# aantropov/Sailor

Measured on AMD Instinct MI355X. Metric: lit Mpixels/s (K0+K1 tile light cull + K2 PBR shade over per-tile lists), higher is better.
Workload: dtype f32; 1 GPU; C3: 3840x2160, 65536 point+spot lights, 16x16 tiles (240x135), cull + PBR shade; width=3840, height=2160, lights=65536, parallelism=tile-row bands x1, partition=whole frame

## Files before the change

sailor_amd/csrc/light_cull.hip:

```cpp
#include "common.h"
#include "light_record.h"
#include <vector>

#define BANDS_PER_BLOCK 24
#define MAX_BANDS_PER_BLOCK 256
#define QCAP 128
#define GROUP 4
#define CAPG 2048
#define GROUP_OVERFLOW 0xFFFFFFFFu
#define GROUP_OVERFLOW_LISTED 0xFFFFFFFEu
#define GROUP_LISTED 0x40000000u
#define HEAVY_MIN_FRAME 512
#define HEAVY_MIN_BAND 384
#define HEAVY_MAX 96
#define CHUNK 512

#define PACK_TILES 64
#define SEL_LIGHTS 1024
#define CL_STEPS (CAPG / 4 / 64)

#define BAND_FORM_MAX_TILES 12000

struct CullLayout {
    int Tx, Ty, bandRows, bandTiles, numBands, words, groupsX, groupsY, numGroups, packBlocks;
// ... 354 lines not shown
        x = L->worldPosition[0]; y = L->worldPosition[1]; z = L->worldPosition[2]; radius = L->bounds[0];
        type = L->type;
    }
}
__device__ __forceinline__ float4 select_view(const SelectArgs& a, const float x, const float y, const float z, const float radius)
{
    float4 p = glsl_mul(a.view, x, y, z, 1.0f);
    const float w = p.w;
    p.x = p.x / w; p.y = p.y / w; p.z = p.z / w;
    p.z = p.z * -1.0f;
    return make_float4(p.x, p.y, p.z, radius);
}

__global__ __launch_bounds__(256) void k0_band_count(const SelectArgs a)
{
    __shared__ float4 sPl[2];
    __shared__ uint32_t sCnt[4][4];
    const int lane = threadIdx.x & 63, wave = threadIdx.x >> 6;
    const uint32_t b = blockIdx.x;
    if (threadIdx.x == 0) {
        Frustum4 f;
        frustum_from_rect(a.invProj, 0.0f, (float)(a.tileRow0 * TILE), (float)(a.Tx * TILE), (float)((a.tileRow0 + a.bandRows) * TILE), a.vpW, a.vpH, f);
        sPl[0] = make_float4(f.n[2][0], f.n[2][1], f.n[2][2], 0.0f);
        sPl[1] = make_float4(f.n[3][0], f.n[3][1], f.n[3][2], 0.0f);
    }
    float4 lv[4];
    uint32_t type[4];
#pragma unroll
    for (int k = 0; k < 4; k++) {
        const int j = (int)b * SEL_LIGHTS + k * 256 + (int)threadIdx.x;
        lv[k] = make_float4(0.0f, 0.0f, 0.0f, 0.0f);
        type[k] = 1u;
        if (j < a.N) {
            float x, y, z, radius;
            if (a.prepStaged) {
                const float4* L = reinterpret_cast<const float4*>(a.lights + j);
                const float4 q0 = L[0], q1 = L[1], q2 = L[2], q3 = L[3], q4 = L[4], q5 = L[5], q6 = L[6];
                x = q1.x; y = q1.y; z = q1.z; radius = q6.x;
                type[k] = __float_as_uint(q0.x);
                a.prepPosRadius[j] = make_float4(x, y, z, radius);
                a.prepType[j] = type[k];
                if (!a.stageSelectedOnly) {
                    float4 o0, o1, o2, o3, o4;
                    stage_light_record(q0, q1, q2, q3, q4, q5, q6, o0, o1, o2, o3, o4);
                    float4* o = a.prepStaged + (size_t)j * LREC;
                    o[0] = o0; o[1] = o1; o[2] = o2; o[3] = o3; o[4] = o4;
                }
            } else select_load(a, j, x, y, z, radius, type[k]);
            lv[k] = select_view(a, x, y, z, radius);
        }
    }
    __syncthreads();
#pragma unroll
    for (int k = 0; k < 4; k++) {
        const int j = (int)b * SEL_LIGHTS + k * 256 + (int)threadIdx.x;
        const bool valid = j < a.N;
        const float r = lv[k].w;
        const float m = a.planeMargin * ((fabsf(lv[k].x) + fabsf(lv[k].y)) + (fabsf(lv[k].z) + fabsf(r)));
        const bool inFront = (lv[k].z - r) > m;
        const float thr = -(r + m);
        const bool keepAlways = valid && (type[k] == 0u || !inFront);
        const float4 nA = sPl[0], nB = sPl[1];
        const bool out = dot3f(nA.x, nA.y, nA.z, lv[k].x, lv[k].y, lv[k].z) < thr || dot3f(nB.x, nB.y, nB.z, lv[k].x, lv[k].y, lv[k].z) < thr;
        const unsigned long long keep = __ballot(keepAlways || (valid && !out));
        if (lane == 0) { a.keep[(size_t)b * 16u + (uint32_t)(4 * k + wave)] = keep; sCnt[k][wave] = (uint32_t)__popcll(keep); }
    }
    __syncthreads();
    if (threadIdx.x == 0) {
        uint32_t total = 0u;
#pragma unroll
        for (int k = 0; k < 4; k++)
#pragma unroll
            for (int w = 0; w < 4; w++) total += sCnt[k][w];
        a.state[2u + b] = total;
    }
}

__global__ __launch_bounds__(256) void k0_band_scatter(const SelectArgs a)
{
    __shared__ uint32_t sPart[4];
    const int lane = threadIdx.x & 63, wave = __builtin_amdgcn_readfirstlane((int)(threadIdx.x >> 6));
    const uint32_t b = blockIdx.x;
    unsigned long long keep[4];
    uint32_t before[4], total = 0u;
#pragma unroll
    for (int k = 0; k < 4; k++) {
        before[k] = total;
#pragma unroll
        for (int w = 0; w < 4; w++) {
            const unsigned long long m = a.keep[(size_t)b * 16u + (uint32_t)(4 * k + w)];
            const uint32_t c = (uint32_t)__popcll(m);
            if (w == wave) keep[k] = m;
            if (w < wave) before[k] += c;
            total += c;
        }
    }
    uint32_t acc = 0u;
    for (uint32_t i = threadIdx.x; i < b; i += 256u) acc += a.state[2u + i];
#pragma unroll
    for (int d = 32; d > 0; d >>= 1) acc += (uint32_t)__shfl_xor((int)acc, d, 64);
    if (lane == 0) sPart[wave] = acc;
    __syncthreads();
    const uint32_t base = (sPart[0] + sPart[1]) + (sPart[2] + sPart[3]);
    if (b == gridDim.x - 1u && threadIdx.x == 0) a.state[0] = base + total;
#pragma unroll
    for (int k = 0; k < 4; k++) {
        if ((keep[k] >> lane) & 1ull) {
            const uint32_t c = base + before[k] + (uint32_t)__popcll(keep[k] & lanemask_lt());
            const int j = (int)b * SEL_LIGHTS + k * 256 + (int)threadIdx.x;
            float x, y, z, radius;
            uint32_t type;
            if (a.prepStaged) {
                const float4 pr = a.prepPosRadius[j];
                x = pr.x; y = pr.y; z = pr.z; radius = pr.w;
                type = a.prepType[j];
            } else select_load(a, j, x, y, z, radius, type);
            a.lightView[c] = select_view(a, x, y, z, radius);
            a.lightType[c] = type;
            a.lightMap[c] = (uint32_t)j;
            if (a.prepStaged && a.stageSelectedOnly) {
                const float4* L = reinterpret_cast<const float4*>(a.lights + j);
                float4 o0, o1, o2, o3, o4;
                stage_light_record(L[0], L[1], L[2], L[3], L[4], L[5], L[6], o0, o1, o2, o3, o4);
                float4* o = a.prepStaged + (size_t)j * LREC;
                o[0] = o0; o[1] = o1; o[2] = o2; o[3] = o3; o[4] = o4;
            }
        }
    }
}

#define LDS_K01_PREPARE (2 * MAX_BANDS_PER_BLOCK * 16)
#ifndef CULL_SGPR_CAP_PREPARE
#define CULL_SGPR_CAP_PREPARE 96
#endif
__global__ __launch_bounds__(256) __attribute__((amdgpu_num_sgpr(CULL_SGPR_CAP_PREPARE))) void k01_prepare(PrepareArgs a)
{
    __shared__ __attribute__((aligned(16))) unsigned char lds[LDS_K01_PREPARE];
    const int b = (int)blockIdx.x;
    if (b == 0 && threadIdx.x == 0) a.heavy[0] = 0u;
    if (b < a.lightRoleBlocks) k0_lights(b, lds, a);
    else if (b < a.lightRoleBlocks + a.frustumBlocks) k1_tile_frusta(b - a.lightRoleBlocks, a);
    else k1_tile_setup(b - a.lightRoleBlocks - a.frustumBlocks, lds, a);
}

__device__ __forceinline__ uint64_t lanemask_lt()
{
    const uint32_t lane = threadIdx.x & 63;
    return lane == 0 ? 0ull : (~0ull >> (64 - lane));
}

#define WAVE_SYNC() __builtin_amdgcn_fence(__ATOMIC_ACQ_REL, "workgroup")

#define GL_WPT 4
__global__ __launch_bounds__(256) void k1_group_lists(const unsigned long long* __restrict__ masks, const unsigned long long* __restrict__ dirWords,
                                                       int stride, int groupsX, uint32_t* __restrict__ groupCount, uint32_t* __restrict__ groupList,
                                                       uint32_t* __restrict__ heavy, uint32_t heavyMin, const uint32_t* __restrict__ selCount)
{
    __shared__ uint32_t sW[4];
    const int g = (int)blockIdx.y * groupsX + (int)blockIdx.x, lane = threadIdx.x & 63, wave = threadIdx.x >> 6;
    const unsigned long long* __restrict__ c = masks + (size_t)blockIdx.x * stride;
    const unsigned long long* __restrict__ r = masks + (size_t)(groupsX + (int)blockIdx.y) * stride;
    const int words = selCount ? min((int)(((*selCount + 63u) / 64u + 1u) & ~1u), stride) : stride;
    uint32_t* __restrict__ list = groupList + (size_t)g * CAPG;
    uint32_t base = 0;
    for (int w0 = 0; w0 < words; w0 += 256 * GL_WPT) {
        const int wFirst = w0 + (int)threadIdx.x * GL_WPT;
        unsigned long long m[GL_WPT], dm[GL_WPT];
        uint32_t cnt = 0;
        if (wFirst + GL_WPT <= words && (words & (GL_WPT - 1)) == 0) {
            const ulonglong2* c2 = reinterpret_cast<const ulonglong2*>(c + wFirst);
            const ulonglong2* r2 = reinterpret_cast<const ulonglong2*>(r + wFirst);
            const ulonglong2* d2 = reinterpret_cast<const ulonglong2*>(dirWords + wFirst);
#pragma unroll
            for (int j = 0; j < GL_WPT / 2; j++) {
                const ulonglong2 cv = c2[j], rv = r2[j], dv = d2[j];
                m[2 * j] = cv.x & rv.x; m[2 * j + 1] = cv.y & rv.y;
                dm[2 * j] = dv.x; dm[2 * j + 1] = dv.y;
            }
        } else {
#pragma unroll
            for (int j = 0; j < GL_WPT; j++) {
                const int w = wFirst + j;
                m[j] = 0ull; dm[j] = 0ull;
                if (w < words) {
                    m[j] = c[w] & r[w];
                    dm[j] = dirWords[w];
                }
            }
        }
#pragma unroll
        for (int j = 0; j < GL_WPT; j++) cnt += (uint32_t)__popcll(m[j]);
        uint32_t incl = cnt;
#pragma unroll
        for (int d = 1; d < 64; d <<= 1) {
            const uint32_t v = (uint32_t)__shfl_up((int)incl, d);
            if (lane >= d) incl += v;
        }
        if (lane == 63) sW[wave] = incl;
        __syncthreads();
        uint32_t before = 0, total = 0;
#pragma unroll
        for (int k = 0; k < 4; k++) { const uint32_t v = sW[k]; before += (k < wave) ? v : 0u; total += v; }
        uint32_t pos = base + before + incl - cnt;
#pragma unroll
        for (int j = 0; j < GL_WPT; j++) {
            const uint32_t first = (uint32_t)(wFirst + j) * 64u;
            unsigned long long mm = m[j];
            const unsigned long long dd = dm[j];
            while (mm != 0ull) {
                const int bit = __builtin_ctzll(mm);
                mm &= mm - 1ull;
                if (pos < CAPG) list[pos] = (first + (uint32_t)bit) | (uint32_t)((dd >> bit) & 1ull) << 31;
                pos++;
            }
        }
        base += total;
        __syncthreads();
    }
    if (threadIdx.x == 0) {
        uint32_t word = base > CAPG ? GROUP_OVERFLOW : base;
        if (base > heavyMin) {
            const uint32_t slot = atomicAdd(&heavy[0], 1u);
            if (slot < (uint32_t)HEAVY_MAX) {
                heavy[1u + slot] = (uint32_t)g;
                word = word != GROUP_OVERFLOW ? (word | GROUP_LISTED) : GROUP_OVERFLOW_LISTED;
            }
        }
        groupCount[g] = word;
    }
}

__device__ __forceinline__ uint32_t wave_incl_scan_u32(uint32_t v)
{
    asm volatile("s_nop 1\n\t"
                 "v_add_u32_dpp %0, %0, %0 row_shr:1 row_mask:0xf bank_mask:0xf bound_ctrl:0\n\t"
                 "s_nop 1\n\t"
                 "v_add_u32_dpp %0, %0, %0 row_shr:2 row_mask:0xf bank_mask:0xf bound_ctrl:0\n\t"
                 "s_nop 1\n\t"
                 "v_add_u32_dpp %0, %0, %0 row_shr:4 row_mask:0xf bank_mask:0xf bound_ctrl:0\n\t"
                 "s_nop 1\n\t"
                 "v_add_u32_dpp %0, %0, %0 row_shr:8 row_mask:0xf bank_mask:0xf bound_ctrl:0\n\t"
                 "s_nop 1\n\t"
                 "v_add_u32_dpp %0, %0, %0 row_bcast:15 row_mask:0xa bank_mask:0xf\n\t"
                 "s_nop 1\n\t"
                 "v_add_u32_dpp %0, %0, %0 row_bcast:31 row_mask:0xc bank_mask:0xf\n\t"
                 "s_nop 1"
                 : "+v"(v));
    return v;
}

#define GLW_ROWS 4
#define GLW_Q 256
template <bool EXACT>
__global__ __launch_bounds__(256) void k1_group_lists_wide(const unsigned long long* __restrict__ masks, const unsigned long long* __restrict__ dirWords,
                                                            int stride, int groupsX, uint32_t* __restrict__ groupCount, uint32_t* __restrict__ groupList,
                                                            const uint32_t* __restrict__ dirFlag, const uint32_t* __restrict__ selCount)
{
    const int words = (!EXACT && selCount) ? min((int)(((*selCount + 63u) / 64u + 1u) & ~1u), stride) : stride;
    __shared__ __attribute__((aligned(16))) unsigned long long sRow[2][GLW_ROWS][128];
    const bool anyDir = *dirFlag != 0u;
    __shared__ unsigned long long sQBits[4][GLW_Q];
    __shared__ uint32_t sQWord[4][GLW_Q];
    const int lane = threadIdx.x & 63, wave = threadIdx.x >> 6;
    const int blocksX = (groupsX + 3) / 4;
    const int gy = (int)blockIdx.x / blocksX, gx = ((int)blockIdx.x % blocksX) * 4 + wave;
    const bool mine = gx < groupsX;
    const int g = gy * groupsX + (mine ? gx : groupsX - 1);
    const unsigned long long* __restrict__ c = masks + (size_t)(mine ? gx : groupsX - 1) * stride;
    const unsigned long long* __restrict__ r = masks + (size_t)(groupsX + gy) * stride;
    uint32_t* __restrict__ list = groupList + (size_t)g * CAPG;
    unsigned long long* qBits = sQBits[wave];
    uint32_t* qWord = sQWord[wave];
    const int rows = (words + 127) / 128, steps = (rows + GLW_ROWS - 1) / GLW_ROWS;
    const ulonglong2 zero2 = { 0ull, 0ull };
    auto load2 = [&](const unsigned long long* __restrict__ m, int row) {
        const int w = row * 128 + lane * 2;
        if (EXACT) return *reinterpret_cast<const ulonglong2*>(m + (row < rows ? w : lane * 2));
        return w < words ? *reinterpret_cast<const ulonglong2*>(m + w) : zero2;
    };
    uint32_t base = 0;
    uint32_t qHead = 0, qTail = 0;
    auto drain = [&](uint32_t n) {
        const uint32_t qi = (qHead + (uint32_t)lane) & (GLW_Q - 1);
        const bool have = (uint32_t)lane < n;
        unsigned long long mm = have ? qBits[qi] : 0ull;
        const uint32_t w = have ? qWord[qi] : 0u;
        const unsigned long long dd = (have && anyDir) ? dirWords[w] : 0ull;
        const uint32_t cnt = (uint32_t)__popcll(mm);
        const uint32_t incl = wave_incl_scan_u32(cnt);
        uint32_t pos = base + incl - cnt;
        const uint32_t first = w * 64u;
        while (mm != 0ull) {
            const int bit = __builtin_ctzll(mm);
            mm &= mm - 1ull;
            if (pos < CAPG) list[pos] = (first + (uint32_t)bit) | (uint32_t)((dd >> bit) & 1ull) << 31;
            pos++;
        }
        base += (uint32_t)__builtin_amdgcn_readlane((int)incl, 63);
        qHead += n;
    };
    ulonglong2 cNext[GLW_ROWS], rNext;
#pragma unroll
    for (int k = 0; k < GLW_ROWS; k++) cNext[k] = load2(c, k);
    rNext = load2(r, wave);
    for (int s = 0; s < steps; s++) {
        ulonglong2 cv[GLW_ROWS];
#pragma unroll
        for (int k = 0; k < GLW_ROWS; k++) cv[k] = cNext[k];
        *reinterpret_cast<ulonglong2*>(&sRow[s & 1][wave][lane * 2]) = rNext;
#pragma unroll
        for (int k = 0; k < GLW_ROWS; k++) cNext[k] = load2(c, (s + 1) * GLW_ROWS + k);
        rNext = load2(r, (s + 1) * GLW_ROWS + wave);
        __syncthreads();
        if (!mine) continue;
#pragma unroll
        for (int k = 0; k < GLW_ROWS; k++) {
            const ulonglong2 rv = *reinterpret_cast<const ulonglong2*>(&sRow[s & 1][k][lane * 2]);
            const unsigned long long m0 = cv[k].x & rv.x, m1 = cv[k].y & rv.y;
            const unsigned long long b0 = __ballot(m0 != 0ull), b1 = __ballot(m1 != 0ull);
            if ((b0 | b1) == 0ull) continue;
            const unsigned long long lt = lanemask_lt();
            const uint32_t i0 = qTail + (uint32_t)__popcll(b0 & lt) + (uint32_t)__popcll(b1 & lt);
            const uint32_t w = (uint32_t)((s * GLW_ROWS + k) * 128 + lane * 2);
            if (m0 != 0ull) { qBits[i0 & (GLW_Q - 1)] = m0; qWord[i0 & (GLW_Q - 1)] = w; }
            const uint32_t i1 = i0 + (m0 != 0ull ? 1u : 0u);
            if (m1 != 0ull) { qBits[i1 & (GLW_Q - 1)] = m1; qWord[i1 & (GLW_Q - 1)] = w + 1u; }
            qTail += (uint32_t)__popcll(b0) + (uint32_t)__popcll(b1);
            while (qTail - qHead >= 64u) { WAVE_SYNC(); drain(64u); WAVE_SYNC(); }
        }
    }
    if (mine) {
        if (qTail != qHead) { WAVE_SYNC(); drain(qTail - qHead); }
        if (lane == 0) groupCount[g] = base > CAPG ? GROUP_OVERFLOW : base;
    }
}

struct TileCtx {
    float n[4][3];
    float cx, cy, cz, zNear, zFar;
};

__device__ __forceinline__ unsigned long long tile_test_mask(const TileCtx& t, const float4 lv)
{
    const float r = lv.w;
    unsigned long long rej = __ballot(lv.z - r > t.zNear) | __ballot(lv.z + r < t.zFar);
#pragma unroll
    for (int k = 0; k < 4; k++) rej |= __ballot(dot3f(t.n[k][0], t.n[k][1], t.n[k][2], lv.x, lv.y, lv.z) < -r);
    return ~rej;
}
__device__ __forceinline__ bool tile_test(const TileCtx& t, const float4 lv)
{
    const float r = lv.w;
    if (lv.z - r > t.zNear || lv.z + r < t.zFar) return false;
#pragma unroll
    for (int k = 0; k < 4; k++)
        if (dot3f(t.n[k][0], t.n[k][1], t.n[k][2], lv.x, lv.y, lv.z) < -r) return false;
    return true;
}

__device__ __forceinline__ float tile_impact(const TileCtx& t, const float4 lv)
{
    const float dx = lv.x - t.cx, dy = lv.y - t.cy, dz = lv.z - t.cz;
    return sqrtf(dot3f(dx, dy, dz, dx, dy, dz));
}

__device__ __forceinline__ void wave_append(bool pass, uint32_t j, uint32_t& count, uint32_t* sIdx)
{
    const uint64_t mask = __ballot(pass);
    const uint32_t pos = count + (uint32_t)__popcll(mask & lanemask_lt());
// ... 289 lines not shown
    uint32_t (*sIdxAll)[CAND] = reinterpret_cast<uint32_t (*)[CAND]>(lds);
    float (*sImpAll)[CAND] = reinterpret_cast<float (*)[CAND]>(lds + 4 * CAND * 4);
    if (blockIdx.x == 0 && blockIdx.y == 0 && threadIdx.x == 0) *a.dirFlag = 0u;
    const int gx = (int)blockIdx.x, tyLocal = (int)blockIdx.y;
    const int wave = __builtin_amdgcn_readfirstlane((int)(threadIdx.x >> 6)), lane = threadIdx.x & 63;
    const int tx = gx * GROUP + wave;
    if (tx >= a.Tx) return;
    const int bandTile = tyLocal * a.Tx + tx;
    TileCtx t;
    load_tile_ctx(a.tileInfo, bandTile, t);
    uint32_t count = 0;
    for (int base = 0; base < a.N && count < CAND; base += 64) {
        const int j = base + lane;
        test_candidates(t, a.lightView, a.lightType, j < a.N, (uint32_t)j, count, sIdxAll[wave]);
    }
    const uint32_t n = count < CAND ? count : CAND;
    if (lane == 0) publish_tile(a, bandTile, n < KEEP ? n : KEEP);
    emit_list<false>(t, n, sIdxAll[wave], sImpAll[wave], a.lightView, a.tileLists + (size_t)bandTile * KEEP, nullptr);
}

template <bool SEL>
__device__ __forceinline__ void block_select(const CullArgs& a, const int firstBandTile, const uint32_t* sCnt, uint32_t (*sIdxAll)[CAND], float (*sImpAll)[CAND], uint32_t* sFlags)
{
    const uint32_t k = threadIdx.x, lane = threadIdx.x & 63;
    const float4* __restrict__ lightView = a.lightView;
    uint32_t mine[4];
    float imp[4];
#pragma unroll
    for (int w = 0; w < 4; w++) {
        const uint32_t n = sCnt[w];
        mine[w] = 0u; imp[w] = 0.0f;
        if (n <= (uint32_t)KEEP) continue;
        const float4* ti = a.tileInfo + (size_t)(firstBandTile + w) * 4;
        const float cx = ti[0].w, cy = ti[1].w, cz = (ti[3].w + ti[2].w) * 0.5f;
        if (k < n) {
            mine[w] = sIdxAll[w][k];
            if (!(mine[w] & 0x80000000u)) {
                const float4 lv = lightView[mine[w] & 0x7FFFFFFFu];
                const float dx = lv.x - cx, dy = lv.y - cy, dz = lv.z - cz;
                imp[w] = sqrtf(dot3f(dx, dy, dz, dx, dy, dz));
            }
            sImpAll[w][k] = imp[w];
        } else if (k < (uint32_t)CAND) reinterpret_cast<uint32_t*>(sImpAll[w])[k] = 0xFFFFFFFFu;
        if (__ballot(k < n && imp[w] != imp[w]) != 0ull && lane == 0) sFlags[w] = 1u;
    }
    __syncthreads();
#pragma unroll
    for (int w = 0; w < 4; w++) {
        const uint32_t n = sCnt[w];
        if (n <= (uint32_t)KEEP) continue;
        uint32_t* __restrict__ out = a.tileLists + (size_t)(firstBandTile + w) * KEEP;
        if (sFlags[w] != 0u) {
            if (threadIdx.x < 64) {
                TileCtx t;
                load_tile_ctx(a.tileInfo, firstBandTile + w, t);
                emit_list<SEL>(t, n, sIdxAll[w], sImpAll[w], lightView, out, a.lightMap);
            }
        } else if (k < n) {
            const uint32_t rank = rank_among(sImpAll[w], n, k, imp[w]);
            if (rank < KEEP) { const uint32_t i = mine[w] & 0x7FFFFFFFu; out[rank] = SEL ? a.lightMap[i] : i; }
        }
    }
}

#ifndef CULL_SGPR_CAP
#define CULL_SGPR_CAP 80
#endif
template <bool COOP, bool SEL>
__global__ __launch_bounds__(256) __attribute__((amdgpu_num_sgpr(CULL_SGPR_CAP))) void k1_tile_cull(const CullArgs a)
{
    __shared__ __attribute__((aligned(16))) unsigned char lds[LDS_K1_TILE_CULL];
    __shared__ uint32_t sCnt[8];
    float4* sLV = reinterpret_cast<float4*>(lds);
    uint32_t* sE = reinterpret_cast<uint32_t*>(lds + CHUNK * 20 - CHUNK * 4);
    uint32_t (*sIdxAll)[CAND] = reinterpret_cast<uint32_t (*)[CAND]>(lds + CHUNK * 20);
    float (*sImpAll)[CAND] = reinterpret_cast<float (*)[CAND]>(lds + CHUNK * 20 + 4 * CAND * 4);
    const float4* __restrict__ lightView = a.lightView;
    const int N = a.N, Tx = a.Tx, groupsX = a.groupsX;
    const int gx = (int)blockIdx.x, tyLocal = (int)blockIdx.y - a.headRows;
    if (blockIdx.x == 0 && blockIdx.y == 0 && threadIdx.x == 0) *a.dirFlag = 0u;
    if (tyLocal < 0) {
        const uint32_t hb = blockIdx.y * (uint32_t)groupsX + blockIdx.x;
        if ((hb >> 4) >= min(a.heavy[0], (uint32_t)HEAVY_MAX)) return;
        const int hg = (int)a.heavy[1u + (hb >> 4)];
        const int row = (hg / groupsX) * GROUP + (int)((hb >> 2) & 3u);
        if (row >= a.bandRows) return;
        PROF_T(0);
        cluster_tile<SEL>(a, lds, sCnt, hg % groupsX, row, (int)(hb & 3u));
        PROF_T(3);
        return;
    }
    PROF_T(0);
    const int g = (tyLocal / GROUP) * groupsX + gx;
    const int wave = __builtin_amdgcn_readfirstlane((int)(threadIdx.x >> 6)), lane = threadIdx.x & 63;
    uint32_t* sIdx = sIdxAll[wave];

    const uint32_t* __restrict__ list = a.groupList + (size_t)g * CAPG;
    uint32_t e[CHUNK / 256];
    e[0] = list[threadIdx.x];
    uint32_t gn = a.groupCount[g];
    if (a.headRows > 0 && (gn == GROUP_OVERFLOW_LISTED || (gn != GROUP_OVERFLOW && (gn & GROUP_LISTED)))) return;
    gn = gn >= GROUP_OVERFLOW_LISTED ? GROUP_OVERFLOW : (gn & ~GROUP_LISTED);
#pragma unroll
    for (int k = 1; k < CHUNK / 256; k++) e[k] = (gn != GROUP_OVERFLOW && gn > 256u * k) ? list[threadIdx.x + 256u * k] : 0u;

    const int tx = gx * GROUP + wave;
    const bool active = tx < Tx;
    const int bandTile = tyLocal * Tx + tx;
    TileCtx t;
    if (active) load_tile_ctx(a.tileInfo, bandTile, t);
    uint32_t count = 0;
    if (gn != GROUP_OVERFLOW) {
        for (uint32_t c0 = 0; c0 < gn; c0 += CHUNK) {
            const uint32_t cn = min((uint32_t)CHUNK, gn - c0);
            if (c0) {
                __syncthreads();
#pragma unroll
                for (int k = 0; k < CHUNK / 256; k++) { const uint32_t i = threadIdx.x + 256u * k; e[k] = i < cn ? list[c0 + i] : 0u; }
            }
            float4 lv[CHUNK / 256];
#pragma unroll
            for (int k = 0; k < CHUNK / 256; k++) {
                lv[k] = make_float4(0.0f, 0.0f, 0.0f, 0.0f);
                if (threadIdx.x + 256u * k < cn) lv[k] = lightView[min(e[k] & 0x7FFFFFFFu, (uint32_t)(N - 1))];
            }
#pragma unroll
            for (int k = 0; k < CHUNK / 256; k++) { const uint32_t i = threadIdx.x + 256u * k; if (i < cn) { sE[i] = e[k]; sLV[i] = lv[k]; } }
            __syncthreads();
            if (active) test_staged(t, cn, sE, sLV, count, sIdx);
        }
    } else if (active) {
        walk_tile_masks(t, a, gx, tyLocal, reinterpret_cast<uint32_t*>(sLV) + wave * QCAP, count, sIdx);
    }
    PROF_T(1);
    const uint32_t n = count < CAND ? count : CAND;
    if (active && lane == 0) publish_tile(a, bandTile, n < KEEP ? n : KEEP);
    if (!COOP || gn == GROUP_OVERFLOW) {
        if (active) emit_list<SEL>(t, n, sIdx, sImpAll[wave], lightView, a.tileLists + (size_t)bandTile * KEEP, a.lightMap);
    } else {
        if (lane == 0) sCnt[wave] = n;
        if (threadIdx.x < 4) sCnt[4 + threadIdx.x] = 0u;
        if (active && n <= KEEP) {
            WAVE_SYNC();
            uint32_t* __restrict__ out = a.tileLists + (size_t)bandTile * KEEP;
            for (uint32_t i = lane; i < n; i += 64) { const uint32_t c = sIdx[n - 1 - i] & 0x7FFFFFFFu; out[i] = SEL ? a.lightMap[c] : c; }
        }
        __syncthreads();
        if (((sCnt[0] > (uint32_t)KEEP) | (sCnt[1] > (uint32_t)KEEP)) | ((sCnt[2] > (uint32_t)KEEP) | (sCnt[3] > (uint32_t)KEEP)))
            block_select<SEL>(a, tyLocal * Tx + gx * GROUP, sCnt, sIdxAll, sImpAll, sCnt + 4);
    }
    PROF_T(3);
}

struct PackArgs {
    const uint32_t* tileNum; const uint8_t* tileNum8; const uint32_t* tileLists;
    SailorLightsGrid* grid; uint32_t* culled;
    int Tx, bandRows, bandTiles;
    uint32_t capacity;
};

__global__ __launch_bounds__(256) void k1_pack(const PackArgs a)
{
    __shared__ __attribute__((aligned(16))) uint32_t sBuf[PACK_TILES * KEEP];
    __shared__ uint32_t sPart[4];
    __shared__ uint32_t sPre[PACK_TILES], sNum[PACK_TILES];
    const int lane = threadIdx.x & 63, wave = threadIdx.x >> 6;
    const int t0 = (int)blockIdx.x * PACK_TILES;
    uint32_t num = 0u;
    const int tile = t0 + lane;
    const bool have = wave == 0 && tile < a.bandTiles;
    if (have) num = a.tileNum[tile];
    uint32_t acc = 0u;
    {
        const uint4* __restrict__ v4 = reinterpret_cast<const uint4*>(a.tileNum8);
        const int count4 = t0 / 16;
        for (int i = threadIdx.x; i < count4; i += 1024) {
            uint4 q[4];
#pragma unroll
            for (int k = 0; k < 4; k++) q[k] = i + 256 * k < count4 ? v4[i + 256 * k] : make_uint4(0u, 0u, 0u, 0u);
#pragma unroll
            for (int k = 0; k < 4; k++) {
                const uint32_t w[4] = { q[k].x, q[k].y, q[k].z, q[k].w };
#pragma unroll
                for (int c = 0; c < 4; c++) {
                    acc = __builtin_amdgcn_sad_u8(w[c], 0u, acc);
                }
            }
        }
    }
#pragma unroll
    for (int d = 32; d > 0; d >>= 1) acc += (uint32_t)__shfl_xor((int)acc, d, 64);
    if (lane == 0) sPart[wave] = acc;
    __syncthreads();
    const uint32_t baseSum = (sPart[0] + sPart[1]) + (sPart[2] + sPart[3]);
    if (wave == 0) {
        uint32_t tincl = num;
#pragma unroll
        for (int d = 1; d < 64; d <<= 1) {
            const uint32_t u = (uint32_t)__shfl_up((int)tincl, d);
            if (lane >= d) tincl += u;
        }
        sPre[lane] = tincl - num;
        sNum[lane] = num;
        const uint32_t offset = 1u + baseSum + tincl - num;
        if (have) {
            const uint32_t fit = offset >= a.capacity ? 0u : min(num, a.capacity - offset);
            a.grid[tile].offset = offset;
            a.grid[tile].num = fit;
        }
        const bool last = t0 + PACK_TILES >= a.bandTiles;
        if (last && lane == 63) {
            const uint32_t tot = baseSum + tincl;
            a.culled[0] = a.capacity ? min(tot, a.capacity - 1u) : 0u;
        }
    }
    __syncthreads();
    {
        const int j = threadIdx.x >> 2, q = threadIdx.x & 3;
        const uint32_t n = sNum[j], pre = sPre[j];
        const uint4* __restrict__ src = reinterpret_cast<const uint4*>(a.tileLists + (size_t)(t0 + j) * KEEP) + q * 8;
        uint4 v[8];
#pragma unroll
        for (int k = 0; k < 8; k++) if ((uint32_t)(32 * q + 4 * k) < n) v[k] = src[k];
#pragma unroll
        for (int k = 0; k < 8; k++) {
            const uint32_t i = (uint32_t)(32 * q + 4 * k);
            if (i < n) {
                uint32_t* d = sBuf + pre + i;
                d[0] = v[k].x;
                if (i + 1u < n) d[1] = v[k].y;
                if (i + 2u < n) d[2] = v[k].z;
                if (i + 3u < n) d[3] = v[k].w;
            }
        }
    }
    __syncthreads();
    const uint32_t total = sPre[PACK_TILES - 1] + sNum[PACK_TILES - 1];
    for (uint32_t i = threadIdx.x; i < total; i += 256u) {
        const uint32_t d = 1u + baseSum + i;
        if (d < a.capacity) a.culled[d] = sBuf[i];
    }
}

__global__ void k_grid_rebase(SailorLightsGrid* grid, int T, uint32_t base)
{
    const int i = blockIdx.x * blockDim.x + threadIdx.x;
    if (i < T) grid[i].offset += base;
}

static bool band_valid(int W, int H, const SailorBand* b)
{
    if (!b) return false;
    const int Ty = (H - 1) / TILE + 1;
    if (b->tileRowBegin < 0 || b->tileRowEnd > Ty || b->tileRowBegin > b->tileRowEnd) return false;
    int lo = H - TILE * b->tileRowEnd, hi = H - TILE * b->tileRowBegin;
    if (lo < 0) lo = 0;
    if (hi > H) hi = H;
    if (hi < lo) hi = lo;
    return b->fbRowBegin == lo && b->fbRowCount == hi - lo;
}

static int band_form_max_tiles()
{
    static const int v = [] { const char* e = getenv("SAILOR_BAND_FORM_TILES"); return e ? atoi(e) : -1; }();
    return v;
}
static bool layout_has_hint(const CullLayout& L, const int lightsCapacity)
{
    if (L.bandRows >= L.Ty || L.bandTiles <= 0) return false;
    const int limit = band_form_max_tiles();
    if (limit >= 0) return L.bandTiles <= limit;
    return L.bandTiles <= BAND_FORM_MAX_TILES || lightsCapacity < 131072;
}

static int launch_pack(SailorHipContext* ctx, const CullLayout& L, char* ws, SailorLightsGrid* dLightsGrid, uint32_t* dCulledLights, size_t culledCapacity)
{
    PackArgs ka;
    ka.tileNum = (const uint32_t*)(ws + L.offTileNum); ka.tileNum8 = (const uint8_t*)(ws + L.offTileNum8); ka.tileLists = (const uint32_t*)(ws + L.offTileLists);
    ka.grid = dLightsGrid; ka.culled = dCulledLights;
    ka.Tx = L.Tx; ka.bandRows = L.bandRows; ka.bandTiles = L.bandTiles;
    ka.capacity = (uint32_t)(culledCapacity > 0xFFFFFFFFull ? 0xFFFFFFFFull : culledCapacity);
    sailor_launch(ctx, k1_pack, dim3(L.packBlocks), dim3(256), ka);
    SAILOR_CHECK_LAUNCH(ctx, "k1_pack");
    return SAILOR_HIP_OK;
}

extern "C" {

int sailor_hip_band_is_valid(int32_t width, int32_t height, const SailorBand* band)
{
    return (width > 0 && height > 0 && band_valid(width, height, band)) ? 1 : 0;
}

size_t sailor_hip_light_cull_workspace_size(int32_t width, int32_t height, int32_t lightsCapacity, const SailorBand* band)
{
    if (width <= 0 || height <= 0 || lightsCapacity < 0) return 0;
    SailorBand whole;
    if (!band) { sailor_hip_band_whole_frame(width, height, &whole); band = &whole; }
    if (!band_valid(width, height, band)) return 0;
    return make_layout(width, height, lightsCapacity, *band).total;
}

int sailor_hip_light_cull(SailorHipContext* ctx, const SailorUboFrameData* frame, const SailorLightCullPushConstants* pc,
                          const SailorLightShaderData* dLights, const float* dLinearDepth,
                          SailorLightsGrid* dLightsGrid, uint32_t* dCulledLights, size_t culledCapacity,
                          void* dWorkspace, size_t workspaceBytes, const SailorBand* band, uint32_t flags)
{
    return sailor_hip_light_cull_prepared(ctx, frame, pc, dLights, dLinearDepth, dLightsGrid, dCulledLights, culledCapacity, dWorkspace, workspaceBytes, band, flags,
                                          nullptr, 0);
}

int sailor_hip_light_cull_prepared(SailorHipContext* ctx, const SailorUboFrameData* frame, const SailorLightCullPushConstants* pc,
                                   const SailorLightShaderData* dLights, const float* dLinearDepth,
                                   SailorLightsGrid* dLightsGrid, uint32_t* dCulledLights, size_t culledCapacity,
                                   void* dWorkspace, size_t workspaceBytes, const SailorBand* band, uint32_t flags,
                                   const void* dPreparedLights, int32_t preparedCapacity)
{
    if (!ctx || !frame || !pc || !dLinearDepth || !dLightsGrid || !dCulledLights || !dWorkspace) return SAILOR_HIP_ERR_INVALID_ARGUMENT;
    const int W = pc->viewportSize[0], H = pc->viewportSize[1], N = pc->lightsNum;
    if (W <= 0 || H <= 0 || N < 0 || (N > 0 && !dLights && !dPreparedLights)) return SAILOR_HIP_ERR_INVALID_ARGUMENT;
    if (dPreparedLights && (preparedCapacity < N || ((uintptr_t)dPreparedLights & 15))) return SAILOR_HIP_ERR_INVALID_ARGUMENT;
    if ((flags & SAILOR_CULL_PREPARE_LIGHTS) && (!dPreparedLights || (N > 0 && (!dLights || ((uintptr_t)dLights & 15))))) return SAILOR_HIP_ERR_INVALID_ARGUMENT;
    if (N > 0x3FFFFFFF) return SAILOR_HIP_ERR_UNSUPPORTED;
    if (frame->viewportSize[0] != W || frame->viewportSize[1] != H) return SAILOR_HIP_ERR_UNSUPPORTED;
    SailorBand whole;
    if (!band) { sailor_hip_band_whole_frame(W, H, &whole); band = &whole; }
    if (!band_valid(W, H, band)) return SAILOR_HIP_ERR_INVALID_ARGUMENT;
    const CullLayout L = make_layout(W, H, N, *band);
    if (pc->numTiles[0] != L.Tx || pc->numTiles[1] != L.Ty) return SAILOR_HIP_ERR_INVALID_ARGUMENT;
    if (workspaceBytes < L.total) return SAILOR_HIP_ERR_WORKSPACE_TOO_SMALL;
    if (culledCapacity < 1 || culledCapacity < (size_t)L.bandTiles * KEEP) return SAILOR_HIP_ERR_INVALID_ARGUMENT;
    if ((unsigned long long)L.bandTiles * KEEP > 0x7FFFFFFFull) return SAILOR_HIP_ERR_UNSUPPORTED;
    if (((uintptr_t)dWorkspace & 255) != 0) return SAILOR_HIP_ERR_INVALID_ARGUMENT;
    SAILOR_TRY_HIP(ctx, hipSetDevice(ctx->device));

    hipStream_t s = ctx->stream;
    char* ws = (char*)dWorkspace;

    if (L.bandTiles == 0) {
        SAILOR_TRY_HIP(ctx, hipMemsetAsync(dCulledLights, 0, 4, s));
        return SAILOR_HIP_OK;
    }

    const float p00 = fabsf(frame->projection[0]), p11 = fabsf(frame->projection[5]);
    const bool sane = p00 > 1e-2f && p11 > 1e-2f && p00 < 1e4f && p11 < 1e4f;
    const bool brute = (flags & SAILOR_CULL_BRUTE_FORCE) || !sane || N < 512;

    PrepareArgs pa;
    memcpy(pa.view.m, frame->view, 64);
    memcpy(pa.invProj.m, frame->invProjection, 64);
    pa.lights = dLights; pa.depth = dLinearDepth;
    pa.soaPosRadius = nullptr; pa.soaType = nullptr;
    pa.prepPosRadius = nullptr; pa.prepType = nullptr; pa.prepStaged = nullptr;
    if (dPreparedLights) {
        const void *pr = nullptr, *ty = nullptr, *st = nullptr;
        sailor_hip_prepared_lights_views(preparedCapacity, dPreparedLights, &pr, &ty, &st);
        if (flags & SAILOR_CULL_PREPARE_LIGHTS) {
            pa.prepPosRadius = (float4*)pr; pa.prepType = (uint32_t*)ty; pa.prepStaged = (float4*)st;
        } else { pa.soaPosRadius = (const float4*)pr; pa.soaType = (const uint32_t*)ty; }
    }
    pa.lightView = (float4*)(ws + L.offLightView); pa.lightType = (uint32_t*)(ws + L.offLightType); pa.tileInfo = (float4*)(ws + L.offTileInfo);
    uint32_t* selState = (uint32_t*)(ws + L.offSelState);
    const bool select = !brute && L.bandRows < L.Ty && !(flags & SAILOR_CULL_NO_BAND_SELECT) && ((flags & SAILOR_CULL_BAND_SELECT) || N >= 131072);
    pa.selCount = nullptr;
    if (select) {
        SelectArgs sa;
        memcpy(sa.view.m, frame->view, 64);
        memcpy(sa.invProj.m, frame->invProjection, 64);
        sa.lights = dLights; sa.soaPosRadius = pa.soaPosRadius; sa.soaType = pa.soaType;
        sa.prepPosRadius = pa.prepPosRadius; sa.prepType = pa.prepType; sa.prepStaged = pa.prepStaged;
        sa.lightView = pa.lightView; sa.lightType = pa.lightType; sa.lightMap = (uint32_t*)(ws + L.offLightMap); sa.state = selState;
        sa.keep = (unsigned long long*)(ws + L.offSelKeep);
        sa.N = N; sa.vpW = frame->viewportSize[0]; sa.vpH = frame->viewportSize[1]; sa.Tx = L.Tx; sa.tileRow0 = band->tileRowBegin; sa.bandRows = L.bandRows;
        sa.planeMargin = 1e-3f;
        sa.stageSelectedOnly = (flags & SAILOR_CULL_PREPARE_SELECTED) ? 1 : 0;
        sailor_launch(ctx, k0_band_count, dim3((unsigned)L.selBlocks), dim3(256), sa);
        SAILOR_CHECK_LAUNCH(ctx, "k0_band_count");
        sailor_launch(ctx, k0_band_scatter, dim3((unsigned)L.selBlocks), dim3(256), sa);
        SAILOR_CHECK_LAUNCH(ctx, "k0_band_scatter");
        pa.selCount = selState;
        pa.prepPosRadius = nullptr; pa.prepType = nullptr; pa.prepStaged = nullptr;
    }
    pa.masks = (unsigned long long*)(ws + L.offMasks); pa.dirWords = (unsigned long long*)(ws + L.offDirWords);
    pa.N = N; pa.words = L.words;
    pa.lightBlocks = (N + 255) / 256;
    pa.numBands = brute ? 0 : L.numBands;
    const int perBlock = (pa.lightBlocks >= 1024 || (flags & SAILOR_CULL_INTERVAL_MASKS)) ? MAX_BANDS_PER_BLOCK : BANDS_PER_BLOCK;
    const int splits = brute ? 1 : (L.numBands + perBlock - 1) / perBlock;
    pa.bandsPerBlock = brute ? 0 : (L.numBands + splits - 1) / splits;
    pa.lightRoleBlocks = pa.lightBlocks * splits;
    pa.intervals = (!brute && splits == 1 && (pa.lightBlocks >= 1024 || (flags & SAILOR_CULL_INTERVAL_MASKS))) ? 1 : 0;
    pa.stripsPerRow = (L.Tx + 16 * SETUP_STRIPS - 1) / (16 * SETUP_STRIPS);
    pa.setupBlocks = pa.stripsPerRow * L.bandRows;
    pa.frustumBlocks = (L.bandTiles + 255) / 256;
    pa.vpW = frame->viewportSize[0]; pa.vpH = frame->viewportSize[1]; pa.W = W; pa.H = H; pa.Tx = L.Tx; pa.Ty = L.Ty;
    pa.tileRow0 = band->tileRowBegin; pa.bandRow0 = band->fbRowBegin; pa.bandRows = L.bandRows; pa.groupsX = L.groupsX;
    pa.vecOK = (((uintptr_t)dLinearDepth & 15) == 0 && (W & 3) == 0) ? 1 : 0;
    pa.rawDepth = (flags & SAILOR_CULL_RAW_DEPTH) ? 1 : 0;
    pa.zNearCam = frame->cameraZNearZFar[0];
    pa.planeMargin = 1e-3f;
    pa.dirFlag = (uint32_t*)(ws + L.offDirFlag);
    pa.heavy = (uint32_t*)(ws + L.offHeavy);
    sailor_launch(ctx, k01_prepare, dim3(pa.lightRoleBlocks + pa.frustumBlocks + pa.setupBlocks), dim3(256), pa);
    SAILOR_CHECK_LAUNCH(ctx, "k01_prepare");

    CullArgs ca;
    ca.lightView = pa.lightView; ca.lightType = pa.lightType; ca.tileInfo = pa.tileInfo; ca.masks = pa.masks;
    ca.groupCount = (const uint32_t*)(ws + L.offGroupCount); ca.groupList = (const uint32_t*)(ws + L.offGroupList);
    ca.tileNum = (uint32_t*)(ws + L.offTileNum); ca.tileNum8 = (uint8_t*)(ws + L.offTileNum8); ca.tileLists = (uint32_t*)(ws + L.offTileLists);
    ca.dirFlag = pa.dirFlag;
    ca.N = N; ca.words = L.words; ca.Tx = L.Tx; ca.groupsX = L.groupsX; ca.bandRows = L.bandRows;
    ca.heavy = (const uint32_t*)(ws + L.offHeavy); ca.headRows = 0;
    ca.lightMap = select ? (const uint32_t*)(ws + L.offLightMap) : nullptr; ca.selCount = pa.selCount;
    if (brute) {
        sailor_launch(ctx, k1_tile_cull_brute, dim3(L.groupsX, L.bandRows), dim3(256), ca);
        SAILOR_CHECK_LAUNCH(ctx, "k1_tile_cull<brute>");
    } else {
        const bool wide = L.words >= 4096 && (L.words & 1) == 0;
        if (wide)
        {
            const dim3 wideGrid((unsigned)(((L.groupsX + 3) / 4) * L.groupsY));
            if (L.words % (128 * GLW_ROWS) == 0 && !select)
                sailor_launch(ctx, k1_group_lists_wide<true>, wideGrid, dim3(256), pa.masks, pa.dirWords, L.words, L.groupsX, (uint32_t*)(ws + L.offGroupCount),
                                   (uint32_t*)(ws + L.offGroupList), (const uint32_t*)(ws + L.offDirFlag), (const uint32_t*)nullptr);
            else
                sailor_launch(ctx, k1_group_lists_wide<false>, wideGrid, dim3(256), pa.masks, pa.dirWords, L.words, L.groupsX, (uint32_t*)(ws + L.offGroupCount),
                                   (uint32_t*)(ws + L.offGroupList), (const uint32_t*)(ws + L.offDirFlag), pa.selCount);
        }
        else {
            sailor_launch(ctx, k1_group_lists, dim3(L.groupsX, L.groupsY), dim3(256), pa.masks, pa.dirWords, L.words, L.groupsX, (uint32_t*)(ws + L.offGroupCount),
                               (uint32_t*)(ws + L.offGroupList), (uint32_t*)(ws + L.offHeavy), (uint32_t)(L.bandRows * 2 > L.Ty ? HEAVY_MIN_FRAME : HEAVY_MIN_BAND), pa.selCount);
            ca.headRows = (16 * HEAVY_MAX + L.groupsX - 1) / L.groupsX;
        }
        SAILOR_CHECK_LAUNCH(ctx, wide ? "k1_group_lists_wide" : "k1_group_lists");
        const bool coop = !wide;
        const dim3 cgrid(L.groupsX, ca.headRows + L.bandRows);
        if (coop) { if (select) sailor_launch(ctx, k1_tile_cull<true, true>, cgrid, dim3(256), ca); else sailor_launch(ctx, k1_tile_cull<true, false>, cgrid, dim3(256), ca); }
        else { if (select) sailor_launch(ctx, k1_tile_cull<false, true>, cgrid, dim3(256), ca); else sailor_launch(ctx, k1_tile_cull<false, false>, cgrid, dim3(256), ca); }
        SAILOR_CHECK_LAUNCH(ctx, "k1_tile_cull");
    }
    if (flags & SAILOR_CULL_DEFER_PACK) return SAILOR_HIP_OK;
    return launch_pack(ctx, L, ws, dLightsGrid, dCulledLights, culledCapacity);
}

int sailor_hip_light_cull_pack(SailorHipContext* ctx, int32_t width, int32_t height, int32_t lightsCapacity, const SailorBand* band, const void* dWorkspace,
                               SailorLightsGrid* dLightsGrid, uint32_t* dCulledLights, size_t culledCapacity)
{
    if (!ctx || !dWorkspace || !dLightsGrid || !dCulledLights || width <= 0 || height <= 0 || lightsCapacity < 0) return SAILOR_HIP_ERR_INVALID_ARGUMENT;
    SailorBand whole;
    if (!band) { sailor_hip_band_whole_frame(width, height, &whole); band = &whole; }
    if (!band_valid(width, height, band)) return SAILOR_HIP_ERR_INVALID_ARGUMENT;
    const CullLayout L = make_layout(width, height, lightsCapacity, *band);
    if (culledCapacity < 1 || culledCapacity < (size_t)L.bandTiles * KEEP) return SAILOR_HIP_ERR_INVALID_ARGUMENT;
    if (((uintptr_t)dWorkspace & 255) != 0) return SAILOR_HIP_ERR_INVALID_ARGUMENT;
    SAILOR_TRY_HIP(ctx, hipSetDevice(ctx->device));
    if (L.bandTiles == 0) {
        SAILOR_TRY_HIP(ctx, hipMemsetAsync(dCulledLights, 0, 4, ctx->stream));
        return SAILOR_HIP_OK;
    }
    return launch_pack(ctx, L, (char*)dWorkspace, dLightsGrid, dCulledLights, culledCapacity);
}

int sailor_hip_light_cull_tile_lists(int32_t width, int32_t height, int32_t lightsCapacity, const SailorBand* band, const void* dWorkspace,
                                     const uint32_t** outTileNum, const uint32_t** outTileLists)
{
    if (!dWorkspace || width <= 0 || height <= 0 || lightsCapacity < 0) return SAILOR_HIP_ERR_INVALID_ARGUMENT;
    SailorBand whole;
    if (!band) { sailor_hip_band_whole_frame(width, height, &whole); band = &whole; }
    if (!band_valid(width, height, band)) return SAILOR_HIP_ERR_INVALID_ARGUMENT;
    const CullLayout L = make_layout(width, height, lightsCapacity, *band);
    if (outTileNum) *outTileNum = (const uint32_t*)((const char*)dWorkspace + L.offTileNum);
    if (outTileLists) *outTileLists = (const uint32_t*)((const char*)dWorkspace + L.offTileLists);
    return SAILOR_HIP_OK;
}

__global__ __launch_bounds__(256) void k_linearize_depth(const float* __restrict__ raw, float* __restrict__ out, size_t count, float zNear, int vec)
{
    const size_t stride = (size_t)gridDim.x * 256;
    if (vec) {
        const size_t n4 = count / 4;
        const float4* __restrict__ r4 = reinterpret_cast<const float4*>(raw);
        float4* __restrict__ o4 = reinterpret_cast<float4*>(out);
        for (size_t i = (size_t)blockIdx.x * 256 + threadIdx.x; i < n4; i += stride) {
            const float4 d = r4[i];
            o4[i] = make_float4(-(-zNear / d.x), -(-zNear / d.y), -(-zNear / d.z), -(-zNear / d.w));
        }
        for (size_t i = n4 * 4 + (size_t)blockIdx.x * 256 + threadIdx.x; i < count; i += stride) out[i] = -(-zNear / raw[i]);
    } else {
        for (size_t i = (size_t)blockIdx.x * 256 + threadIdx.x; i < count; i += stride) out[i] = -(-zNear / raw[i]);
    }
}

int sailor_hip_linearize_depth(SailorHipContext* ctx, const SailorUboFrameData* frame, const float* dRawDepth, float* dLinearDepth, int32_t width, int32_t rows)
{
    if (!ctx || !frame || !dRawDepth || !dLinearDepth || width <= 0 || rows < 0) return SAILOR_HIP_ERR_INVALID_ARGUMENT;
    const size_t count = (size_t)width * (size_t)rows;
    if (count == 0) return SAILOR_HIP_OK;
    SAILOR_TRY_HIP(ctx, hipSetDevice(ctx->device));
    const int vec = ((((uintptr_t)dRawDepth | (uintptr_t)dLinearDepth) & 15) == 0) ? 1 : 0;
    size_t blocks = (count / 4 + 255) / 256;
    if (blocks > 256 * 32) blocks = 256 * 32;
    if (blocks < 1) blocks = 1;
    hipLaunchKernelGGL(k_linearize_depth, dim3((unsigned)blocks), dim3(256), 0, ctx->stream, dRawDepth, dLinearDepth, count, frame->cameraZNearZFar[0], vec);
    SAILOR_CHECK_LAUNCH(ctx, "k_linearize_depth");
    return SAILOR_HIP_OK;
}

const uint32_t* sailor_hip_light_cull_tile_order(int32_t width, int32_t height, int32_t lightsCapacity, const SailorBand* band, const void* dWorkspace)
{
    if (!dWorkspace || width <= 0 || height <= 0 || lightsCapacity < 0) return nullptr;
    SailorBand whole;
    if (!band) { sailor_hip_band_whole_frame(width, height, &whole); band = &whole; }
    if (!band_valid(width, height, band)) return nullptr;
    const CullLayout L = make_layout(width, height, lightsCapacity, *band);
    if (!layout_has_hint(L, lightsCapacity)) return nullptr;
    return (const uint32_t*)((const char*)dWorkspace + L.offTileNum8);
}

int sailor_hip_light_cull_band_selection(int32_t width, int32_t height, int32_t lightsNum, const SailorBand* band, const void* dWorkspace,
                                         const uint32_t** outSelectedCount, const uint32_t** outLightMap)
{
    if (!dWorkspace || width <= 0 || height <= 0 || lightsNum < 0) return SAILOR_HIP_ERR_INVALID_ARGUMENT;
    SailorBand whole;
    if (!band) { sailor_hip_band_whole_frame(width, height, &whole); band = &whole; }
    if (!band_valid(width, height, band)) return SAILOR_HIP_ERR_INVALID_ARGUMENT;
    const CullLayout L = make_layout(width, height, lightsNum, *band);
    if (outSelectedCount) *outSelectedCount = (const uint32_t*)((const char*)dWorkspace + L.offSelState);
    if (outLightMap) *outLightMap = (const uint32_t*)((const char*)dWorkspace + L.offLightMap);
    return SAILOR_HIP_OK;
}

int sailor_hip_light_cull_diagnostics(SailorHipContext* ctx, int32_t width, int32_t height, int32_t lightsNum, const SailorBand* band,
                                      const void* dWorkspace, uint64_t* out8)
{
    if (!ctx || !dWorkspace || !out8 || width <= 0 || height <= 0 || lightsNum < 0) return SAILOR_HIP_ERR_INVALID_ARGUMENT;
    SailorBand whole;
    if (!band) { sailor_hip_band_whole_frame(width, height, &whole); band = &whole; }
    if (!band_valid(width, height, band)) return SAILOR_HIP_ERR_INVALID_ARGUMENT;
    const CullLayout L = make_layout(width, height, lightsNum, *band);
    std::vector<unsigned long long> masks((size_t)L.numBands * L.words);
    std::vector<uint32_t> counts((size_t)L.numGroups);
    SAILOR_TRY_HIP(ctx, hipStreamSynchronize(ctx->stream));
    SAILOR_TRY_HIP(ctx, hipMemcpy(masks.data(), (const char*)dWorkspace + L.offMasks, masks.size() * 8, hipMemcpyDeviceToHost));
    SAILOR_TRY_HIP(ctx, hipMemcpy(counts.data(), (const char*)dWorkspace + L.offGroupCount, counts.size() * 4, hipMemcpyDeviceToHost));
    uint64_t bits = 0, colBits = 0, sum = 0, over = 0, longest = 0;
    for (size_t i = 0; i < masks.size(); i++) {
        const uint64_t c = (uint64_t)__builtin_popcountll(masks[i]);
        bits += c;
        if (i < (size_t)L.groupsX * L.words) colBits += c;
    }
    for (uint32_t c : counts) {
        if (c >= GROUP_OVERFLOW_LISTED) { over++; continue; }
        c &= ~GROUP_LISTED;
        sum += c;
        if (c > longest) longest = c;
    }
    out8[0] = (uint64_t)L.numBands; out8[1] = bits; out8[2] = (uint64_t)L.numGroups; out8[3] = sum;
    out8[4] = over; out8[5] = longest; out8[6] = (uint64_t)L.words; out8[7] = colBits;
    return SAILOR_HIP_OK;
}

int sailor_hip_light_grid_rebase(SailorHipContext* ctx, SailorLightsGrid* dLightsGrid, int32_t numTiles, uint32_t globalBase)
{
    if (!ctx || !dLightsGrid || numTiles < 0) return SAILOR_HIP_ERR_INVALID_ARGUMENT;
    if (numTiles == 0 || globalBase == 0) return SAILOR_HIP_OK;
    SAILOR_TRY_HIP(ctx, hipSetDevice(ctx->device));
    hipLaunchKernelGGL(k_grid_rebase, dim3((numTiles + 255) / 256), dim3(256), 0, ctx->stream, dLightsGrid, numTiles, globalBase);
    SAILOR_CHECK_LAUNCH(ctx, "k_grid_rebase");
    return SAILOR_HIP_OK;
}

}
```

Before: 50290 Mpixels/s.

## Depth-prefilter group light lists and cull tiles with one wave per tile

The group-list builder now computes a conservative depth range for each 4x4 tile group from the tile info. It stages candidate lights in LDS and drops lights that fall outside that depth range (directional entries are always kept) before writing the group list, so per-tile culling has fewer candidates. For whole-frame, non-select, non-wide layouts, a new 64-thread one-wave-per-tile cull kernel replaces the 256-thread cooperative kernel, with its own heavy-group head rows. The cost is extra barriers, LDS staging and lightView loads in the list builder, plus a different occupancy profile for the cull.

```diff
diff --git a/sailor_amd/csrc/light_cull.hip b/sailor_amd/csrc/light_cull.hip
--- a/sailor_amd/csrc/light_cull.hip
+++ b/sailor_amd/csrc/light_cull.hip
@@ -530,17 +530,41 @@
 #define WAVE_SYNC() __builtin_amdgcn_fence(__ATOMIC_ACQ_REL, "workgroup")
 
 #define GL_WPT 4
+#define GL_STAGE 2048
 __global__ __launch_bounds__(256) void k1_group_lists(const unsigned long long* __restrict__ masks, const unsigned long long* __restrict__ dirWords,
                                                        int stride, int groupsX, uint32_t* __restrict__ groupCount, uint32_t* __restrict__ groupList,
-                                                       uint32_t* __restrict__ heavy, uint32_t heavyMin, const uint32_t* __restrict__ selCount)
+                                                       uint32_t* __restrict__ heavy, uint32_t heavyMin, const uint32_t* __restrict__ selCount,
+                                                       const float4* __restrict__ lightView, const float4* __restrict__ tileInfo, int Tx, int bandRows)
 {
     __shared__ uint32_t sW[4];
+    __shared__ uint32_t sKeep[2][4];
+    __shared__ uint32_t sStage[GL_STAGE];
     const int g = (int)blockIdx.y * groupsX + (int)blockIdx.x, lane = threadIdx.x & 63, wave = threadIdx.x >> 6;
     const unsigned long long* __restrict__ c = masks + (size_t)blockIdx.x * stride;
     const unsigned long long* __restrict__ r = masks + (size_t)(groupsX + (int)blockIdx.y) * stride;
     const int words = selCount ? min((int)(((*selCount + 63u) / 64u + 1u) & ~1u), stride) : stride;
     uint32_t* __restrict__ list = groupList + (size_t)g * CAPG;
+    float ZN = -__builtin_inff(), ZF = __builtin_inff();
+    {
+        bool nanN = false, nanF = false;
+        const float* __restrict__ ti = reinterpret_cast<const float*>(tileInfo);
+#pragma unroll
+        for (int ry = 0; ry < GROUP; ry++) {
+#pragma unroll
+            for (int cx = 0; cx < GROUP; cx++) {
+                const int ty = (int)blockIdx.y * GROUP + ry, tx = (int)blockIdx.x * GROUP + cx;
+                if (ty < bandRows && tx < Tx) {
+                    const float zn = ti[(size_t)(ty * Tx + tx) * 16 + 11], zf = ti[(size_t)(ty * Tx + tx) * 16 + 15];
+                    if (zn != zn) nanN = true; else ZN = fmaxf(ZN, zn);
+                    if (zf != zf) nanF = true; else ZF = fminf(ZF, zf);
+                }
+            }
+        }
+        if (nanN) ZN = __builtin_inff();
+        if (nanF) ZF = -__builtin_inff();
+    }
     uint32_t base = 0;
+    uint32_t parity = 0;
     for (int w0 = 0; w0 < words; w0 += 256 * GL_WPT) {
         const int wFirst = w0 + (int)threadIdx.x * GL_WPT;
         unsigned long long m[GL_WPT], dm[GL_WPT];
@@ -579,20 +603,44 @@
         uint32_t before = 0, total = 0;
 #pragma unroll
         for (int k = 0; k < 4; k++) { const uint32_t v = sW[k]; before += (k < wave) ? v : 0u; total += v; }
-        uint32_t pos = base + before + incl - cnt;
-#pragma unroll
-        for (int j = 0; j < GL_WPT; j++) {
-            const uint32_t first = (uint32_t)(wFirst + j) * 64u;
-            unsigned long long mm = m[j];
-            const unsigned long long dd = dm[j];
-            while (mm != 0ull) {
-                const int bit = __builtin_ctzll(mm);
-                mm &= mm - 1ull;
-                if (pos < CAPG) list[pos] = (first + (uint32_t)bit) | (uint32_t)((dd >> bit) & 1ull) << 31;
-                pos++;
-            }
-        }
-        base += total;
+        uint32_t pos = before + incl - cnt;
+        for (uint32_t p0 = 0; p0 < total; p0 += GL_STAGE) {
+            const uint32_t pEnd = p0 + GL_STAGE;
+#pragma unroll
+            for (int j = 0; j < GL_WPT; j++) {
+                const uint32_t first = (uint32_t)(wFirst + j) * 64u;
+                while (m[j] != 0ull && pos < pEnd) {
+                    const int bit = __builtin_ctzll(m[j]);
+                    m[j] &= m[j] - 1ull;
+                    sStage[pos - p0] = (first + (uint32_t)bit) | (uint32_t)((dm[j] >> bit) & 1ull) << 31;
+                    pos++;
+                }
+            }
+            __syncthreads();
+            const uint32_t n = min((uint32_t)GL_STAGE, total - p0);
+            for (uint32_t i0 = 0; i0 < n; i0 += 256u) {
+                const uint32_t i = i0 + threadIdx.x;
+                uint32_t e = 0u;
+                bool keep = false;
+                if (i < n) {
+                    e = sStage[i];
+                    const float4 lv = lightView[e & 0x7FFFFFFFu];
+                    const float rad = lv.w;
+                    keep = (int)e < 0 || !(lv.z - rad > ZN || lv.z + rad < ZF);
+                }
+                const unsigned long long km = __ballot(keep);
+                if (lane == 0) sKeep[parity][wave] = (uint32_t)__popcll(km);
+                __syncthreads();
+                uint32_t kb = 0, kt = 0;
+#pragma unroll
+                for (int k = 0; k < 4; k++) { const uint32_t v = sKeep[parity][k]; kb += (k < wave) ? v : 0u; kt += v; }
+                const uint32_t o = base + kb + (uint32_t)__popcll(km & lanemask_lt());
+                if (keep && o < CAPG) list[o] = e;
+                base += kt;
+                parity ^= 1u;
+            }
+            __syncthreads();
+        }
         __syncthreads();
     }
     if (threadIdx.x == 0) {
@@ -1188,6 +1236,60 @@
     PROF_T(3);
 }
 
+#define LDS_K1_TILE_CULL_WAVE (2 * CAND * 4 + QCAP * 4)
+__device__ __forceinline__ void wave_tile(const CullArgs& a, unsigned char* __restrict__ lds, const int tx, const int tyLocal, const bool fromHead)
+{
+    uint32_t* sIdx = reinterpret_cast<uint32_t*>(lds);
+    float* sImp = reinterpret_cast<float*>(lds + CAND * 4);
+    uint32_t* sQ = reinterpret_cast<uint32_t*>(lds + 2 * CAND * 4);
+    const uint32_t lane = threadIdx.x;
+    const float4* __restrict__ lightView = a.lightView;
+    const int gx = tx / GROUP, g = (tyLocal / GROUP) * a.groupsX + gx;
+    const uint32_t* __restrict__ list = a.groupList + (size_t)g * CAPG;
+    uint32_t eCur = list[lane], eNxt = list[64u + lane];
+    uint32_t gn = a.groupCount[g];
+    if (!fromHead && (gn == GROUP_OVERFLOW_LISTED || (gn != GROUP_OVERFLOW && (gn & GROUP_LISTED)))) return;
+    gn = gn >= GROUP_OVERFLOW_LISTED ? GROUP_OVERFLOW : (gn & ~GROUP_LISTED);
+    const uint32_t last = (uint32_t)(a.N - 1);
+    const int bandTile = tyLocal * a.Tx + tx;
+    TileCtx t;
+    load_tile_ctx(a.tileInfo, bandTile, t);
+    uint32_t count = 0;
+    if (gn != GROUP_OVERFLOW) {
+        float4 lvCur = lightView[lane < gn ? min(eCur & 0x7FFFFFFFu, last) : 0u];
+        for (uint32_t base = 0; base < gn && count < CAND; base += 64u) {
+            const uint32_t i = base + lane;
+            const uint32_t eAfter = list[min(i + 128u, (uint32_t)CAPG - 1u)];
+            const float4 lvNxt = lightView[i + 64u < gn ? min(eNxt & 0x7FFFFFFFu, last) : 0u];
+            const unsigned long long mask = __ballot(i < gn) & (__ballot((int)eCur < 0) | tile_test_mask(t, lvCur));
+            wave_append_mask(mask, eCur, count, sIdx);
+            eCur = eNxt; lvCur = lvNxt; eNxt = eAfter;
+        }
+    } else {
+        walk_tile_masks(t, a, gx, tyLocal, sQ, count, sIdx);
+    }
+    const uint32_t n = count < CAND ? count : CAND;
+    if (lane == 0) publish_tile(a, bandTile, n < KEEP ? n : KEEP);
+    emit_list<false>(t, n, sIdx, sImp, lightView, a.tileLists + (size_t)bandTile * KEEP, nullptr);
+}
+
+__global__ __launch_bounds__(64) __attribute__((amdgpu_num_sgpr(CULL_SGPR_CAP), amdgpu_waves_per_eu(8, 8))) void k1_tile_cull_wave(const CullArgs a)
+{
+    __shared__ __attribute__((aligned(16))) unsigned char lds[LDS_K1_TILE_CULL_WAVE];
+    int tx = (int)blockIdx.x, tyLocal = (int)blockIdx.y - a.headRows;
+    if (blockIdx.x == 0 && blockIdx.y == 0 && threadIdx.x == 0) *a.dirFlag = 0u;
+    const bool head = tyLocal < 0;
+    if (head) {
+        const uint32_t hb = blockIdx.y * (uint32_t)a.Tx + blockIdx.x;
+        if ((hb >> 4) >= min(a.heavy[0], (uint32_t)HEAVY_MAX)) return;
+        const int hg = (int)a.heavy[1u + (hb >> 4)];
+        tyLocal = (hg / a.groupsX) * GROUP + (int)((hb >> 2) & 3u);
+        tx = (hg % a.groupsX) * GROUP + (int)(hb & 3u);
+        if (tyLocal >= a.bandRows || tx >= a.Tx) return;
+    }
+    wave_tile(a, lds, tx, tyLocal, head);
+}
+
 struct PackArgs {
     const uint32_t* tileNum; const uint8_t* tileNum8; const uint32_t* tileLists;
     SailorLightsGrid* grid; uint32_t* culled;
@@ -1465,13 +1567,17 @@
         }
         else {
             sailor_launch(ctx, k1_group_lists, dim3(L.groupsX, L.groupsY), dim3(256), pa.masks, pa.dirWords, L.words, L.groupsX, (uint32_t*)(ws + L.offGroupCount),
-                               (uint32_t*)(ws + L.offGroupList), (uint32_t*)(ws + L.offHeavy), (uint32_t)(L.bandRows * 2 > L.Ty ? HEAVY_MIN_FRAME : HEAVY_MIN_BAND), pa.selCount);
+                               (uint32_t*)(ws + L.offGroupList), (uint32_t*)(ws + L.offHeavy), (uint32_t)(L.bandRows * 2 > L.Ty ? HEAVY_MIN_FRAME : HEAVY_MIN_BAND), pa.selCount,
+                               (const float4*)pa.lightView, (const float4*)pa.tileInfo, L.Tx, L.bandRows);
             ca.headRows = (16 * HEAVY_MAX + L.groupsX - 1) / L.groupsX;
         }
         SAILOR_CHECK_LAUNCH(ctx, wide ? "k1_group_lists_wide" : "k1_group_lists");
         const bool coop = !wide;
-        const dim3 cgrid(L.groupsX, ca.headRows + L.bandRows);
-        if (coop) { if (select) sailor_launch(ctx, k1_tile_cull<true, true>, cgrid, dim3(256), ca); else sailor_launch(ctx, k1_tile_cull<true, false>, cgrid, dim3(256), ca); }
+        const bool waveForm = !wide && !select && L.bandRows == L.Ty;
+        if (waveForm) ca.headRows = (16 * HEAVY_MAX + L.Tx - 1) / L.Tx;
+        const dim3 cgrid(waveForm ? L.Tx : L.groupsX, ca.headRows + L.bandRows);
+        if (waveForm) sailor_launch(ctx, k1_tile_cull_wave, cgrid, dim3(64), ca);
+        else if (coop) { if (select) sailor_launch(ctx, k1_tile_cull<true, true>, cgrid, dim3(256), ca); else sailor_launch(ctx, k1_tile_cull<true, false>, cgrid, dim3(256), ca); }
         else { if (select) sailor_launch(ctx, k1_tile_cull<false, true>, cgrid, dim3(256), ca); else sailor_launch(ctx, k1_tile_cull<false, false>, cgrid, dim3(256), ca); }
         SAILOR_CHECK_LAUNCH(ctx, "k1_tile_cull");
     }
```

Result: slower. 48730 Mpixels/s (-3.1%).
